# DanieleTeni/Online-Non-Linear-Centroidal-MPC-with-stability-Guarantees-for-Robust-Locomotion-of-Legged-Robots-

Hardware: AMD Instinct MI355X
Metric: centroidal-MPC solves/sec, N=20 horizon (higher is better)
Workload: dtype f64

## Files before the change

build.py:

```python
import os
import subprocess
import sys

ROOT = os.path.dirname(os.path.abspath(__file__))
PKG = os.path.join(ROOT, "online-non-linear-centroidal-mpc-with-stability-guarantees-for-robust-locomotion-of-legged-robots-_amd")


def _newer(target, sources):
    if not os.path.exists(target):
        return True
    t = os.path.getmtime(target)
    return any(os.path.getmtime(s) > t for s in sources)


CSRC = os.path.join(PKG, "csrc")
KERNEL_DEPS = [os.path.join(CSRC, "cmpc_kernel.hpp"), os.path.join(CSRC, "cmpc_lds_asm.hpp"), os.path.join(CSRC, "cmpc_wave.hpp"),
               os.path.join(ROOT, "include", "cmpc.h")]
RBD_DEPS = [os.path.join(CSRC, "rbd_kernel.hpp"), os.path.join(ROOT, "include", "cmpc_rbd.h")]
DEVICE_UNITS = [os.path.join(CSRC, "cmpc_hip.hip"), os.path.join(CSRC, "wbc_qp.hip"), os.path.join(CSRC, "rbd.hip")]
DEVICE_DEPS = DEVICE_UNITS + KERNEL_DEPS + RBD_DEPS + [
    os.path.join(CSRC, "cmpc_order_fit.h"), os.path.join(ROOT, "include", "cmpc_wbc.h")]
EMU_DIR = os.path.join(ROOT, "tests", "emu")


def _hipcc_lib(out, defines=(), force=False, verbose=False):
    if force or _newer(out, DEVICE_DEPS):
        subprocess.check_call(["hipcc"] + (["-Rpass-analysis=kernel-resource-usage"] if verbose else [])
                              + ["--offload-arch=gfx950", "-O3", "-std=c++17", "-fPIC", "-shared"]
                              + ["-D" + d for d in defines] + ["-o", out] + DEVICE_UNITS)
    return out


def _emu_lib(src, out, defines=(), force=False):
    src, out = os.path.join(EMU_DIR, src), os.path.join(EMU_DIR, out)
    if force or _newer(out, [src, os.path.join(EMU_DIR, "cmpc_emu.cpp")] + KERNEL_DEPS):
        subprocess.check_call(["g++", "-O2", "-std=c++17", "-mfma", "-ffp-contract=off", "-fPIC", "-shared", "-pthread"]
                              + ["-D" + d for d in defines] + ["-o", out, src])
    return out


def build_hip(force=False, verbose=False):
    return _hipcc_lib(os.path.join(PKG, "libcmpc_amd.so"), force=force, verbose=verbose)


def build_hip_profile(force=False):
    return _hipcc_lib(os.path.join(ROOT, "tools", "libcmpc_amd_prof.so"), ["CMPC_PROFILE"], force)


def build_hip_dev(force=False):
    return _hipcc_lib(os.path.join(ROOT, "tools", "libcmpc_amd_dev.so"), ["CMPC_DEV_KNOBS"], force)


def build_hip_no_reuse(force=False, profile=False):
    return _hipcc_lib(os.path.join(ROOT, "tools", "libcmpc_amd_noreuse_prof.so" if profile else "libcmpc_amd_noreuse.so"),
                      ["CMPC_NO_EVAL_REUSE", "CMPC_SEPARATE_STEP"] + (["CMPC_PROFILE"] if profile else []), force)


def build_hip_separate_step(force=False, profile=False):
    return _hipcc_lib(os.path.join(ROOT, "tools", "libcmpc_amd_sepstep_prof.so" if profile else "libcmpc_amd_sepstep.so"),
                      ["CMPC_SEPARATE_STEP"] + (["CMPC_PROFILE"] if profile else []), force)


def build_oracle(force=False):
    out = os.path.join(ROOT, "oracle", "libcmpc_oracle.so")
    deps = [os.path.join(ROOT, "oracle", "cmpc_oracle.c"), os.path.join(ROOT, "include", "cmpc.h")]
    if force or _newer(out, deps):
        subprocess.check_call(["make", "-C", os.path.join(ROOT, "oracle"), "-B", "libcmpc_oracle.so"],
                              stdout=subprocess.DEVNULL)
    return out


def build_emu(force=False):
    return _emu_lib("cmpc_emu.cpp", "libcmpc_emu.so", force=force)


def build_emu_gain(force=False):
    return _emu_lib("cmpc_emu_gain.cpp", "libcmpc_emu_gain.so", force=force)


def build_emu_consts(force=False):
    return _emu_lib("cmpc_emu_consts.cpp", "libcmpc_emu_consts.so", force=force)


def build_emu_gain_consts(force=False):
    return _emu_lib("cmpc_emu_gain_consts.cpp", "libcmpc_emu_gain_consts.so", force=force)


def build_emu_reuse(force=False, reuse=True):
    return _emu_lib("cmpc_emu_reuse.cpp", "libcmpc_emu_reuse.so" if reuse else "libcmpc_emu_noreuse.so",
                    [] if reuse else ["CMPC_NO_EVAL_REUSE"], force)


def build_emu_step(force=False, fused=True):
    return _emu_lib("cmpc_emu_step.cpp", "libcmpc_emu_step.so" if fused else "libcmpc_emu_sepstep.so",
                    [] if fused else ["CMPC_SEPARATE_STEP"], force)


def build_emu_rbd(force=False):
    src, out = os.path.join(EMU_DIR, "rbd_emu.cpp"), os.path.join(EMU_DIR, "librbd_emu.so")
    if force or _newer(out, [src] + RBD_DEPS):
        subprocess.check_call(["g++", "-O2", "-std=c++17", "-mfma", "-ffp-contract=off", "-fPIC", "-shared", "-pthread",
                               "-o", out, src])
    return out


def build_device_unit(force=False):
    src = os.path.join(ROOT, "tests", "gpu_unit", "cmpc_device_unit.hip")
    out = os.path.join(ROOT, "tests", "gpu_unit", "libcmpc_device_unit.so")
    if force or _newer(out, [src] + KERNEL_DEPS):
        subprocess.check_call(["hipcc", "--offload-arch=gfx950", "-O3", "-std=c++17", "-fPIC", "-shared", "-o", out, src])
    return out


def build_tools(force=False):
    outs = []
    for name in ("hbm_calib", "lds_b128_repro"):
        src = os.path.join(ROOT, "tools", "ubench", name + ".hip")
        out = os.path.join(ROOT, "tools", "ubench", name)
        if force or _newer(out, [src]):
            r = subprocess.run(["hipcc", "--offload-arch=gfx950", "-O3", "-o", out, src], capture_output=True, text=True)
            if r.returncode != 0:
                print(f"build_tools: {name} failed to compile (profiling scripts that need it will not run)\n{r.stderr}",
                      file=sys.stderr)
                continue
        outs.append(out)
    return outs


if __name__ == "__main__":
    force = "--force" in sys.argv
    print(build_hip(force, verbose="-v" in sys.argv))
    print(build_oracle(force))
    print(build_emu(force))
    print(build_emu_gain(force))
    print(build_emu_consts(force))
    print(build_emu_gain_consts(force))
    print(build_emu_reuse(force))
    print(build_emu_reuse(force, reuse=False))
    print(build_emu_step(force))
    print(build_emu_step(force, fused=False))
    print(build_emu_rbd(force))
    print(build_device_unit(force))
    print(build_tools(force))
```

online-non-linear-centroidal-mpc-with-stability-guarantees-for-robust-locomotion-of-legged-robots-_amd/csrc/cmpc_kernel.hpp:

```cpp
#pragma once
#include "../../include/cmpc.h"
#include <math.h>
#include <utility>
#ifdef CMPC_HOST_EMU
#include <cstdio>
#include <cstdlib>
#endif

#ifndef CMPC_HOST_EMU
#include <hip/hip_runtime.h>
#define CMPC_DEV __device__ __forceinline__
#define CMPC_LANE ((int)threadIdx.x)
#define CMPC_SYNC() asm volatile("s_waitcnt lgkmcnt(0)" ::: "memory")
#define CMPC_SYNC_GLOBAL() __syncthreads()
#define CMPC_SYNC_WG() asm volatile("s_waitcnt lgkmcnt(0)\n\ts_barrier" ::: "memory")
#define CMPC_WAVE_ID() ((int)__builtin_amdgcn_readfirstlane((int)threadIdx.x >> 6))
static __device__ __forceinline__ double cmpc_bcast(double v, int src) {
  union { double d; int i[2]; } u; u.d = v;
  u.i[0] = __builtin_amdgcn_readlane(u.i[0], src);
  u.i[1] = __builtin_amdgcn_readlane(u.i[1], src);
  return u.d;
}
#define CMPC_BCAST(v, src) cmpc_bcast((v), (src))
typedef double cmpc_v4d __attribute__((ext_vector_type(4)));
#define CMPC_MFMA_F64(a, b, c) __builtin_amdgcn_mfma_f64_16x16x4f64((a), (b), (c), 0, 0, 0)
#include "cmpc_wave.hpp"
#define CMPC_PAIR_OF(M, v, a, b) cmpc_pair_of<M>((v), (a), (b))
#define CMPC_OPAQUE(x) asm volatile("" : "+v"(x))
#define CMPC_OPAQUE_D(x) asm volatile("" : "+v"(x))
#define CMPC_OPAQUE_S(x) asm volatile("" : "+s"(x))
#define CMPC_UNIFORM_INT(x) __builtin_amdgcn_readfirstlane(x)
static __device__ __forceinline__ double cmpc_fresh(double a) { asm volatile("" : "+s"(a)); return a; }
#define CMPC_FRESH_D(x) cmpc_fresh(x)
#ifdef CMPC_FRESH_SPEC
#define SPD(field) cmpc_fresh(CMPC_SPEC_OR_ROW(field))
#else
#define SPD(field) (EVAL_REUSE ? cmpc_fresh(CMPC_SPEC_OR_ROW(field)) : CMPC_SPEC_OR_ROW(field))
#endif
typedef const double __attribute__((address_space(4))) *cmpc_crow_t;
#define CMPC_CROW(p) ((cmpc_crow_t)(p))
static __device__ __forceinline__ cmpc_crow_t cmpc_fresh_row(cmpc_crow_t r) { asm volatile("" : "+s"(r)); return r; }
#define CMPC_ROW_AT(r, i) (cmpc_fresh_row(r)[i])
static __device__ __forceinline__ double cmpc_uniform_d(double v) {
  union { double d; int i[2]; } u; u.d = v;
  int lo, hi;
  asm("s_nop 0\n\tv_readfirstlane_b32 %0, %2\n\tv_readfirstlane_b32 %1, %3\n\ts_nop 1" : "=s"(lo), "=s"(hi) : "v"(u.i[0]), "v"(u.i[1]));
  u.i[0] = lo; u.i[1] = hi;
  return u.d;
}
#ifdef CMPC_NO_UNIFORM_D
#define CMPC_UNIFORM_D(x) (x)
#else
#define CMPC_UNIFORM_D(x) cmpc_uniform_d(x)
#endif
#define CMPC_SCHED_FENCE() __builtin_amdgcn_sched_barrier(0)
#define CMPC_RELANE(x) do { (x) = (int)__builtin_amdgcn_mbcnt_hi(~0u, __builtin_amdgcn_mbcnt_lo(~0u, 0u)) + lane_base; } while (0)
#define CMPC_SYNC_WAVE(w) CMPC_SYNC()
#define CMPC_FENCE_WAVE(w) asm volatile("s_waitcnt vmcnt(0) lgkmcnt(0)" ::: "memory")
#define CMPC_VM_LANDED() __builtin_amdgcn_s_waitcnt(0x0F70)
#define CMPC_ASM_NOTE(text) asm volatile("; " text)
#endif
#ifdef CMPC_HOST_EMU
#define CMPC_SYNC_WAVE(w) emu_barrier_wait(&emu_wave_barrier[(w)])
#define CMPC_FENCE_WAVE(w) emu_barrier_wait(&emu_wave_barrier[(w)])
#define CMPC_SYNC_WG() emu_barrier_wait(&emu_barrier)
#define CMPC_VM_LANDED() do { } while (0)
#define CMPC_ASM_NOTE(text) do { } while (0)
#endif
#ifndef CMPC_RELANE
#define CMPC_RELANE(x) do { } while (0)
#define SPD(field) CMPC_SPEC_OR_ROW(field)
typedef const double *cmpc_crow_t;
#define CMPC_CROW(p) ((cmpc_crow_t)(p))
#define CMPC_ROW_AT(r, i) ((r)[i])
#define CMPC_FRESH_D(x) (x)
#define CMPC_UNIFORM_D(x) (x)
#endif
#define CMPC_CIDX(field) ((int)((__builtin_offsetof(cmpc_spec, field) - __builtin_offsetof(cmpc_spec, delta)) / sizeof(double)))
#define CMPC_SPEC_OR_ROW(field) (CONSTS ? CMPC_ROW_AT(crow, CMPC_CIDX(field)) : sp.field)
static_assert(CMPC_CIDX(relax) == CMPC_NCONST - 1 && CMPC_CIDX(box[2]) == 13 && __builtin_offsetof(cmpc_spec, tol) == __builtin_offsetof(cmpc_spec, relax) + sizeof(double),
              "the row of per-instance constants is the block of cmpc_spec from delta to relax");
#define CMPC_FMA(x, y, z) __builtin_fma((x), (y), (z))
#ifdef CMPC_HOST_EMU
#define CMPC_STEP_MAD(t, b, a) ((a) + (t) * (b))
#else
#define CMPC_STEP_MAD(t, b, a) __builtin_fma((t), (b), (a))
#endif
#ifndef CMPC_OPAQUE_D
#define CMPC_OPAQUE_D(x) do { } while (0)
#endif
#ifndef CMPC_UNIFORM_INT
#define CMPC_UNIFORM_INT(x) (x)
#endif
#ifndef CMPC_OPAQUE_S
#define CMPC_OPAQUE_S(x) do { } while (0)
#endif

#if defined(CMPC_PROFILE) && !defined(CMPC_HOST_EMU)
static __device__ __forceinline__ constexpr int cmpc_retry_class(int slot) {
  return (slot == 11 || slot == 12 || slot == 26 || slot == 0) ? 31
       : (slot == 24 || slot == 25) ? 32
       : (slot == 27) ? 34
       : 33;
}
#define CMPC_TICK(slot) do { long long now_ = clock64(); tprof[slot] += now_ - tlast; \
    if (prof_retry) tprof[cmpc_retry_class(slot)] += now_ - tlast; \
    tlast = now_; } while (0)
#define CMPC_TICK_RESET() do { tlast = clock64(); } while (0)
#define CMPC_RETRY_STAT(slot, n) do { tprof[slot] += (n); } while (0)
#define CMPC_RETRY_MARK(on) do { prof_retry = (on); } while (0)
#define CMPC_RETRY_TRACK 1
#else
#define CMPC_TICK(slot) do { } while (0)
#define CMPC_TICK_RESET() do { } while (0)
#define CMPC_RETRY_MARK(on) do { } while (0)
#define CMPC_RETRY_TRACK 0
#endif
#ifndef CMPC_RETRY_STAT
#define CMPC_RETRY_STAT(slot, n) do { } while (0)
#endif
#ifndef CMPC_STEP_STAT
#define CMPC_STEP_STAT(slot, n) do { } while (0)
#endif
#define CMPC_NPROF 36

namespace cmpc {

struct KArgs {
  cmpc_spec sp;
  int B;
  const double *recs;
  const double *warm;
  const double *state_in;
  double *state_out;
  double *out;
  int32_t *status;
  int32_t *iters;
  double *kkt;
  double *scratch;
  size_t scratch_stride;
  long long *prof;
  double tol_acc, tol_tenth;
};

enum { R_LYAP = 0, R_CZ = 1, R_HWC = 2, R_BOX = 3, R_FRIC = 15 };

constexpr double ACC_FACTOR = 100.0;
constexpr int ACC_ITERS = 8;
inline void fill_levels(KArgs &ka) { ka.tol_acc = ACC_FACTOR * ka.sp.tol; ka.tol_tenth = ka.sp.tol / 10; }
constexpr double STALL_STEP = 1e-7;
constexpr int STALL_ITERS = 6;
constexpr int NOPROG_ITERS = 12;
constexpr double PIV_MIN = 1e-8;
constexpr double PIV_FRAC = 0.1;
constexpr int POLISH_ITERS = 1;
constexpr double MU_INIT = 100.0;
constexpr double MU_FACTOR = 0.1;
constexpr double MU_WARM = 1e-7;
constexpr bool COLD_ROLLOUT = true;
constexpr int RESUME_RECENTRE_ITERS = 20;
constexpr int WAVES_NV8 = 2;
constexpr double GAIN_SIG_CAP = 1e12;
constexpr double GAIN_SIG_CAP_BOX = 2e10;

#ifndef CMPC_NO_DEVICE_CODE
#include "cmpc_lds_asm.hpp"
#endif

#ifndef CMPC_NO_DEVICE_CODE
template <int CNT> CMPC_DEV void lds_read_row(double (&v)[CNT], const double *p) {
  static_assert(CNT == 28 || CNT == 32 || CNT == 36 || CNT == 56, "supported row lengths");
  if constexpr (CNT == 28) lds_read_strided28<1>(v, p);
  else if constexpr (CNT == 32) {
    double a[16], b[16];
    lds_read_strided16<1>(a, p); lds_read_strided16<1>(b, p + 16);
#pragma unroll
    for (int i = 0; i < 16; ++i) { v[i] = a[i]; v[16 + i] = b[i]; }
  } else if constexpr (CNT == 36) {
    double a[18], b[18];
    lds_read_strided18<1>(a, p); lds_read_strided18<1>(b, p + 18);
#pragma unroll
    for (int i = 0; i < 18; ++i) { v[i] = a[i]; v[18 + i] = b[i]; }
  } else {
    double a[28], b[28];
    lds_read_strided28<1>(a, p); lds_read_strided28<1>(b, p + 28);
#pragma unroll
    for (int i = 0; i < 28; ++i) { v[i] = a[i]; v[28 + i] = b[i]; }
  }
}
#endif

template <int NV, int NW> struct Sizes {
  static_assert(NW == 1 || NW == 2, "one or two waves per instance");
  static constexpr int WS = 64 * NW;
  static constexpr int NF = 2 * NV;
  static constexpr int NU = 6 * NV + 8;
  static constexpr int NXA = CMPC_NX + 2 * NV;
  static constexpr int NZ = NU + NXA;
  static constexpr int NI = 15 + 10 * NV;
  static constexpr int NTRI = NZ * (NZ + 1) / 2;
  static constexpr int NH = (NZ + WS - 1) / WS;
  static constexpr int PS = NXA + 1;
  static constexpr int LS = NU + 1;
  static constexpr int NPT = NXA * (NXA + 1) / 2;
};

template <int NV, int NW, bool PIPE> struct LdsMap : Sizes<NV, NW> {
// ... 114 lines not shown
  static constexpr int gG = gL + NU;
  static constexpr int gL1 = gG + NI;
  static constexpr int gPV1 = gL1 + NU;
  static constexpr int STAGE = ((gPV1 + NXA + 7) / 8) * 8;
  static constexpr int rH0 = 0, rH1 = rH0 + NZ, rW0 = rH1 + NZ, rVDV = rW0 + NI, rQ = rVDV + 3 * NF, rPI = rQ + 2;
  static constexpr int RE_STAGE = COMPACT ? ((rPI + 3 + 7) / 8) * 8 : 0;
  static constexpr int state_lam(int N) { return CMPC_NSOL(N, NV); }
  static constexpr int state_s(int N) { return state_lam(N) + (N + 1) * NXA; }
  static constexpr int state_z(int N) { return state_s(N) + (N + 1) * NI; }
  static constexpr int state_mu(int N) { return state_z(N) + (N + 1) * NI; }
  static constexpr int state_fl(int N) { return state_mu(N) + 8; }
  static_assert(state_fl(20) + 2 * 21 == CMPC_NSTATE(20, NV), "layout of include/cmpc.h");
  static size_t scratch_doubles(int N) {
    size_t n = (size_t)(N + 1) * STAGE;
    n += (size_t)(N + 1) * NXA * 4;
    n += (size_t)(N + 1) * NU * 3;
    n += (size_t)(N + 1) * NI * 4;
    n += (size_t)(N + 1) * RE_STAGE;
    return (n + 7) / 8 * 8;
  }
};

#ifndef CMPC_NO_DEVICE_CODE

CMPC_DEV int tri(int i) { return i * (i + 1) / 2; }

typedef double cmpc_v2d __attribute__((vector_size(16)));
struct GArr {
  double *p;
  CMPC_DEV double &operator[](unsigned i) const { return *(double *)((char *)p + (size_t)(i * 8u)); }
  CMPC_DEV cmpc_v2d &pair(unsigned i) const { return *(cmpc_v2d *)((char *)p + (size_t)(i * 16u)); }
};

CMPC_DEV bool consts_row_ok(cmpc_crow_t row) {
  bool ok = true;
  for (int i = 0; i < CMPC_NCONST; ++i) {
    const double v = row[i];
    const bool positive = i == CMPC_CIDX(delta) || i == CMPC_CIDX(g) || (i >= CMPC_CIDX(cz_max) && i <= CMPC_CIDX(foot_width));
    const bool gain = i == CMPC_CIDX(k1) || i == CMPC_CIDX(k2);
    ok = ok && v < INFINITY && v > -INFINITY && (positive ? v > 0.0 : (gain || v >= 0.0));
  }
  return ok;
}

template <int NV, int NW = 1, bool PIPE = false, bool GAIN = false, bool CONSTS = false> struct Solver {
  using D = Dims<NV, NW, PIPE>;
  static constexpr int XCH_DU = 16, XCH_DOUBLES = XCH_DU + 2 * D::NU;
  static_assert(!PIPE || XCH_DOUBLES <= D::P_DOUBLES, "the exchange words fit in the unused P region of the second image");
  static constexpr int XCH_AT = D::LDS_DOUBLES + D::oP;
  static_assert(!PIPE || NW == 1, "the pipelined pair runs the one-wave solver");
  static_assert(!PIPE || (D::oUB + 64 <= D::oBV && D::oUB >= D::oXN1 + D::NXA && !D::GT_FIRST),
                "pair_vectors reads BV / writes XN1 of the image the Riccati wave is working in");
  static constexpr int NF = D::NF, NU = D::NU, NXA = D::NXA, NZ = D::NZ, NI = D::NI, NH = D::NH, WS = D::WS;
  static_assert(NW == 1 || NU <= 64, "the input rows (pivot chains, substitutions) live in the first wave");
#ifdef CMPC_NO_EVAL_REUSE
  static constexpr bool EVAL_REUSE = false;
#else
  static constexpr bool EVAL_REUSE = NV == 4 && NW == 1 && !PIPE && !GAIN && D::GT_FIRST;
#endif
  static constexpr bool RETRY_TRACK_POSSIBLE = NV == 4 && NW == 1 && !PIPE && !GAIN;
  static constexpr int ER_AT = 256;
  static_assert(!RETRY_TRACK_POSSIBLE || (ER_AT >= 3 * NZ + NXA + 3 * NF && ER_AT + 6 * WS <= D::NTRI), "the parked error measures fit the M region");
#ifdef CMPC_SEPARATE_STEP
  static constexpr bool STEP_FUSED = false;
#else
  static constexpr bool STEP_FUSED = RETRY_TRACK_POSSIBLE;
#endif
  static constexpr bool RETRY_TRACK = EVAL_REUSE || STEP_FUSED || (CMPC_RETRY_TRACK && NV == 4 && NW == 1 && !PIPE && !GAIN);

  const KArgs &ka;
  const cmpc_spec &sp;
  double *lds;
  double *ldsR;
  int lane_base = 0;
  GArr gs;
  GArr rec;
  int N, lane;
  int wv = 0;
  GArr gx, glam, gdx, glamn, gu, gdu, gupx, gsl, gz, gds, gdz;
  int lr[NH][6];
  double lg[NH][6];
  double piv_min = PIV_MIN;
  GArr st_in{nullptr};
  long long tprof[CMPC_NPROF] = {0, 0, 0, 0, 0, 0, 0, 0, 0, 0, 0, 0, 0, 0, 0, 0, 0, 0, 0, 0, 0, 0, 0, 0, 0, 0, 0, 0, 0, 0, 0, 0, 0, 0, 0, 0}, tlast = 0;
  bool prof_retry = false;
  double *gain_out = nullptr;
  GArr gbuf{nullptr};
  bool gain_sweep = false;
  cmpc_crow_t crow = nullptr;

  CMPC_DEV Solver(const KArgs &a, double *l, double *g, const double *r)
      : ka(a), sp(a.sp), lds(l), ldsR(l), gs{g}, rec{const_cast<double *>(r)}, N(a.sp.N), lane(CMPC_LANE) {
    if constexpr (NW > 1 || PIPE) wv = CMPC_WAVE_ID();
    if constexpr (NW > 1) lane_base = 64 * wv;
    if constexpr (PIPE) lane &= 63;
    if constexpr (NW == 1 && !PIPE) CMPC_RELANE(lane);
    double *p = g + (size_t)(N + 1) * D::STAGE;
    gx = GArr{p}; p += (size_t)(N + 1) * NXA;
    glam = GArr{p}; p += (size_t)(N + 1) * NXA;
    gdx = GArr{p}; p += (size_t)(N + 1) * NXA;
    glamn = GArr{p}; p += (size_t)(N + 1) * NXA;
    gu = GArr{p}; p += (size_t)(N + 1) * NU;
    gdu = GArr{p}; p += (size_t)(N + 1) * NU;
    gupx = GArr{p}; p += (size_t)(N + 1) * NU;
    gsl = GArr{p}; p += (size_t)(N + 1) * NI;
    gz = GArr{p}; p += (size_t)(N + 1) * NI;
    gds = GArr{p}; p += (size_t)(N + 1) * NI;
    gdz = GArr{p};
  }
  CMPC_DEV GArr stage(int k) const { return GArr{gs.p + (size_t)k * D::STAGE}; }
  CMPC_DEV unsigned restage(int k) const {
    CMPC_OPAQUE_S(k);
    return (unsigned)((N + 1 - k) * D::STAGE + (N + 1) * (4 * NXA + 3 * NU + 4 * NI) + k * D::RE_STAGE);
  }
  CMPC_DEV double &L(int o) const { return lds[o]; }
  CMPC_DEV double &R(int o) const { return ldsR[o]; }
  CMPC_DEV void image(int k) { if constexpr (PIPE) lds = ldsR + (k & 1) * D::LDS_DOUBLES; }
  CMPC_DEV void sync() const {
    if constexpr (PIPE) { CMPC_SYNC_WAVE(wv); }
    else {
#ifdef CMPC_HOST_EMU
      CMPC_SYNC();
#else
      if constexpr (NW == 1) CMPC_SYNC(); else CMPC_SYNC_WG();
#endif
    }
  }
  CMPC_DEV void gsync() const {
    if constexpr (PIPE) { CMPC_FENCE_WAVE(wv); } else { CMPC_SYNC_GLOBAL(); }
  }
  CMPC_DEV void pair_sync() const { if constexpr (PIPE) { CMPC_SYNC_GLOBAL(); } }
  CMPC_DEV bool first_wave() const { return NW == 1 || wv == 0; }

  CMPC_DEV double gam_k(int k, int f) const { return (k == N) ? L(D::oHDR + 22 + f) : L(D::oSR + 17 + f); }
  CMPC_DEV double gam_km1(int f) const { return L(D::oSRP + 17 + f); }
  CMPC_DEV void vert_local(int j, double &vx, double &vy) const {
    const double Lh = SPD(foot_length) * 0.5, Wh = SPD(foot_width) * 0.5;
    const double cx[8] = {Lh, Lh, -Lh, -Lh, Lh, 0.0, -Lh, 0.0};
    const double cy[8] = {Wh, -Wh, -Wh, Wh, 0.0, -Wh, 0.0, Wh};
    vx = cx[j]; vy = cy[j];
  }

  CMPC_DEV static double step_axpy(double a, double t, double b) { return CMPC_STEP_MAD(t, b, a); }
  CMPC_DEV static double step_toward(double c, double t, double d) { return CMPC_STEP_MAD(t, d - c, c); }
  CMPC_DEV static void step_slack(double &s, double &z, double ds, double dz, double ap, double ad, double mu) {
    s = CMPC_STEP_MAD(ap, ds, s);
    const double zn = CMPC_STEP_MAD(ad, dz, z);
    const double lo = mu / s / 1e10, hi = mu / s * 1e10;
    z = fmin(fmax(zn, lo), hi);
  }

  CMPC_DEV void load_stage(int k, bool first = false, double mu = 0.0) {
    static_assert(NXA <= 64 && NU <= 64, "one lane per state / input component");
    constexpr int NIH = (NI + WS - 1) / WS;
    const bool in = k < N;
    const int kn = in ? k + 1 : k, ku = in ? k : N - 1, kp = (k >= 1) ? k - 1 : 0;
    const int ix = (lane < NXA) ? lane : 0, iu = (lane < NU) ? lane : 0, ir = (lane < 19) ? lane : 0;
    bool step = false;
    if constexpr (STEP_FUSED) { if (first) step = CMPC_UNIFORM_INT((int)(L(D::oSTEP_ON) != 0.0)) != 0; }
    double dxv = 0.0, lnv = 0.0, duv = 0.0, dsv[NIH], dzv[NIH];
#pragma unroll
    for (int h = 0; h < NIH; ++h) { dsv[h] = 0.0; dzv[h] = 0.0; }
    if constexpr (STEP_FUSED) {
      if (step) {
        dxv = gdx[k * NXA + ix]; lnv = glamn[k * NXA + ix]; duv = gdu[ku * NU + iu];
#pragma unroll
        for (int h = 0; h < NIH; ++h) {
// ... 1293 lines not shown
          if (!riccati_stage(k) && lane == 0) xch[8 + (j & 1)] = 1.0;
        }
        CMPC_SYNC_WG();
        const bool failed = xch[8 + (j & 1)] != 0.0;
        if (failed) { image(0); CMPC_SYNC_WG(); return false; }
      }
      image(0);
      pair_sync();
      return true;
    }
  }

  enum { OP_MAX = 0, OP_MIN = 1, OP_SUM = 2 };
  CMPC_DEV double across_waves(double v, int op) {
    if constexpr (NW == 1) return v;
    if ((lane & 63) == 0) R(D::oCOLD + 4 + wv) = v;
    sync();
    const double a = R(D::oCOLD + 4), b = R(D::oCOLD + 5);
    sync();
    return (op == OP_MAX) ? fmax(a, b) : (op == OP_MIN) ? fmin(a, b) : a + b;
  }
  template <int M> CMPC_DEV static double bfly_sum(double v) { double a, b; CMPC_PAIR_OF(M, v, a, b); return a + b; }
  template <int M> CMPC_DEV static double bfly_max(double v) { double a, b; CMPC_PAIR_OF(M, v, a, b); return fmax(a, b); }
  template <int M> CMPC_DEV static double bfly_min(double v) { double a, b; CMPC_PAIR_OF(M, v, a, b); return fmin(a, b); }
  CMPC_DEV static double wave_sum(double v) {
    v = bfly_sum<32>(v); v = bfly_sum<16>(v); v = bfly_sum<8>(v); v = bfly_sum<4>(v); v = bfly_sum<2>(v); return bfly_sum<1>(v);
  }
  CMPC_DEV double red_max(double v) {
    v = bfly_max<32>(v); v = bfly_max<16>(v); v = bfly_max<8>(v); v = bfly_max<4>(v); v = bfly_max<2>(v); v = bfly_max<1>(v);
    return across_waves(v, OP_MAX);
  }
  CMPC_DEV double red_min(double v) {
    v = bfly_min<32>(v); v = bfly_min<16>(v); v = bfly_min<8>(v); v = bfly_min<4>(v); v = bfly_min<2>(v); v = bfly_min<1>(v);
    return across_waves(v, OP_MIN);
  }
  CMPC_DEV double red_sum(double v) { return across_waves(wave_sum(v), OP_SUM); }

  CMPC_DEV void vector_sweeps(double mu, double dmu, double &ap, double &ad) {
    if constexpr (PIPE) {
      image(0);
      if (wv == 1) { slack_sweep(mu, ap, ad); return; }
    }
    mu = CMPC_UNIFORM_D(mu); dmu = CMPC_UNIFORM_D(dmu);
    const double m = CMPC_UNIFORM_D(rec[20]), muf = CMPC_UNIFORM_D(rec[21]);
    constexpr int NIH = (NI + WS - 1) / WS;
    const double tau = CMPC_UNIFORM_D(fmax(0.99, 1 - mu));
    const double d_m = CMPC_UNIFORM_D(SPD(delta) / m);
    double lap = 1.0, lad = 1.0;
    double *xdu = ldsR + XCH_AT + XCH_DU;
    constexpr bool MERGE = D::W_MERGE;
    const bool isA = lane < NU;
    const int lb = MERGE ? lane - NU : lane;
    const bool isB = lb >= 0 && lb < NXA;
    gsync();
    int cur = D::oXK, nxt = D::oXN1;
    if (lane < NXA) { L(cur + lane) = 0.0; gdx[lane] = 0.0; }
    sync();
    struct Early { double l0v, l1v, dg, pv0, pv1; };
    struct Late { double gh[3][NH], al[NH], sv[NIH], zv[NIH], gv[NIH], hw0, hw1, hw2, bq; };
    double wa[NXA], wb[MERGE ? 1 : NXA], lam[NU];
    auto load_w = [&](int k) {
      const GArr st = stage(k);
      if constexpr (MERGE) {
        const int lc = (lane < NZ) ? lane : 0;
        const int rb = tri(lc) + NU;
#pragma unroll
        for (int c = 0; c < NXA; ++c) wa[c] = st[D::gM + ((lc < NU || NU + c >= lc) ? tri(NU + c) + lc : rb + c)];
        wb[0] = 0.0;
      } else {
        const int la = (lane < NU) ? lane : 0;
        const int lbc = (lane < NXA) ? lane : 0, rb = tri(NU + lbc) + NU;
#pragma unroll
        for (int c = 0; c < NXA; ++c) wa[c] = st[D::gM + tri(NU + c) + la];
#pragma unroll
        for (int c = 0; c < NXA; ++c) wb[c] = st[D::gM + ((c >= lbc) ? tri(NU + c) + NU + lbc : rb + c)];
      }
    };
    auto load_lam = [&](int k) {
      const GArr st = stage(k);
      const int la = (lane < NU) ? lane : 0;
#pragma unroll
      for (int j = 0; j < NU; ++j) lam[j] = st[D::gM + tri(j) + la];
    };
    auto load_early = [&](int k, Early &w) {
      const GArr st = stage(k);
      const int lb_ = MERGE ? lane - NU : lane;
      const int la = (lane < NU) ? lane : 0, lbc = (lb_ >= 0 && lb_ < NXA) ? lb_ : 0;
      w.l0v = st[D::gL + la]; w.l1v = st[D::gL1 + la]; w.dg = st[D::gM + tri(la) + la];
      w.pv0 = st[D::gPV + lbc]; w.pv1 = st[D::gPV1 + lbc];
    };
    auto load_late = [&](int k, Late &w) {
      const GArr st = stage(k);
#pragma unroll
      for (int r = 0; r < 3; ++r)
#pragma unroll
        for (int h = 0; h < NH; ++h) w.gh[r][h] = st[D::gGH + r * D::GHS + lane + WS * h];
      if constexpr (!PIPE) {
#pragma unroll
        for (int h = 0; h < NH; ++h) { const int c = lane + WS * h; w.al[h] = st[D::gAL + ((c < NZ) ? c : 0)]; }
#pragma unroll
        for (int h = 0; h < NIH; ++h) {
          const int r = lane + WS * h, rc = (r < NI) ? r : 0;
          w.sv[h] = gsl[k * NI + rc]; w.zv[h] = gz[k * NI + rc]; w.gv[h] = st[D::gG + rc];
        }
        w.hw0 = gx[k * NXA + 6]; w.hw1 = gx[k * NXA + 7]; w.hw2 = gx[k * NXA + 8];
      } else {
#pragma unroll
        for (int h = 0; h < NH; ++h) w.al[h] = 0.0;
#pragma unroll
        for (int h = 0; h < NIH; ++h) { w.sv[h] = 0.0; w.zv[h] = 0.0; w.gv[h] = 0.0; }
        w.hw0 = 0.0; w.hw1 = 0.0; w.hw2 = 0.0;
      }
      w.bq = st[D::gB + ((lane < NXA) ? lane : 0)];
    };
#ifndef CMPC_FWD_AHEAD_MASK
#define CMPC_FWD_AHEAD_MASK 7
#endif
    constexpr bool AHEAD = ((CMPC_FWD_AHEAD_MASK) >> (PIPE ? 1 : (NW == 1 ? 0 : 2))) & 1;
    Early sm;
    if constexpr (AHEAD) { load_w(0); CMPC_SCHED_FENCE(); load_early(0, sm); CMPC_SCHED_FENCE(); load_lam(0); CMPC_SCHED_FENCE(); }
    else { sm.l0v = 0.0; sm.l1v = 0.0; sm.dg = 0.0; sm.pv0 = 0.0; sm.pv1 = 0.0; }
    for (int k = 0; k <= N; ++k) {
      CMPC_RELANE(lane); CMPC_OPAQUE(lane);
      const bool hasA = k < N, hasB = k >= 1;
      const int kn = hasA ? k + 1 : k;
      const double gl = rec[(k < N) ? 24 + 19 * k + 17 : 22], gr = rec[(k < N) ? 24 + 19 * k + 18 : 23];
      Late lt;
      load_late(k, lt);
      if constexpr (!AHEAD) { load_w(k); load_early(k, sm); load_lam(k); }
      const double (&gh)[3][NH] = lt.gh;
      const double (&al)[NH] = lt.al, (&sv)[NIH] = lt.sv, (&zv)[NIH] = lt.zv, (&gv)[NIH] = lt.gv;
      const double hw0 = lt.hw0, hw1 = lt.hw1, hw2 = lt.hw2, bq = lt.bq;
      const double l0v = sm.l0v, l1v = sm.l1v, dg = sm.dg, pv0 = sm.pv0, pv1 = sm.pv1;
      CMPC_TICK(16);
      double accA, accB;
      {
        const double *dxv = &L(cur);
        double a0 = 0.0, a1 = 0.0, a2 = 0.0, a3 = 0.0;
        static_assert(NXA % 4 == 0, "unroll by 4");
#pragma unroll
        for (int c = 0; c < NXA; c += 4) {
          a0 += wa[c] * dxv[c]; a1 += wa[c + 1] * dxv[c + 1]; a2 += wa[c + 2] * dxv[c + 2]; a3 += wa[c + 3] * dxv[c + 3];
          if (c % 8 == 4) CMPC_SCHED_FENCE();
        }
        accA = (a0 + a1) + (a2 + a3);
        if constexpr (!MERGE) {
          double b0 = 0.0, b1 = 0.0, b2 = 0.0, b3 = 0.0;
#pragma unroll
          for (int c = 0; c < NXA; c += 4) {
            b0 += wb[c] * dxv[c]; b1 += wb[c + 1] * dxv[c + 1]; b2 += wb[c + 2] * dxv[c + 2]; b3 += wb[c + 3] * dxv[c + 3];
          }
          accB = (b0 + b1) + (b2 + b3);
        } else accB = accA;
      }
      CMPC_OPAQUE_D(accA); CMPC_OPAQUE_D(accB);
      if constexpr (AHEAD) load_w(kn);
      if (hasB && isB) glamn[k * NXA + lb] = pv0 + dmu * pv1 + accB;
      auto slack_dirs = [&](double ldot) {
#pragma unroll
        for (int h = 0; h < NIH; ++h) {
          const int r = lane + WS * h;
          if (r < NI) {
            const double sr_ = sv[h], zr = zv[h], gr_ = gv[h];
            double ds = 0.0, dz = 0.0;
            if (zr != 0.0) {
              ds = -(gr_ + sr_) - jg_dot(r, ldot, &L(cur), &L(D::oUK), hw0, hw1, hw2, gl, gr, muf);
              dz = (mu - sr_ * zr - zr * ds) / sr_;
              if (ds < 0) lap = fmin(lap, -tau * sr_ / ds);
              if (dz < 0) lad = fmin(lad, -tau * zr / dz);
            }
            gds[k * NI + r] = ds; gdz[k * NI + r] = dz;
          }
        }
      };
      double duv = 0.0;
      if (hasA && first_wave()) {
        double treg = isA ? -(l0v + dmu * l1v + accA) : 0.0;
        const double dinv = 1.0 / dg;
#pragma unroll
        for (int j = NU - 1; j >= 0; --j) {
          const double dj = CMPC_BCAST(treg * dinv, j);
          if (lane < j) treg -= lam[j] * dj;
        }
        duv = treg * dinv;
        if (isA) { gdu[k * NU + lane] = duv; L(D::oUK + lane) = duv; }
        if constexpr (PIPE) { if (isA) xdu[(k & 1) * NU + lane] = duv; }
      }
      if constexpr (AHEAD) { load_early(kn, sm); load_lam(kn); }
      if (!hasA) {
        if constexpr (PIPE) { CMPC_SYNC_WG(); break; }
        double part = 0.0;
#pragma unroll
        for (int h = 0; h < NH; ++h) {
          const int c = lane + WS * h;
          if (c >= NU && c < NZ) part += al[h] * L(cur + c - NU);
        }
        slack_dirs(red_sum(part));
        sync();
        break;
      }
      if constexpr (PIPE) CMPC_SYNC_WG();
      double s0 = 0.0, s1 = 0.0, s2 = 0.0, s3 = 0.0;
#pragma unroll
      for (int h = 0; h < NH; ++h) {
        const int c = lane + WS * h;
        const bool in = c < NZ;
        const double z = (c < NU) ? duv : (in ? L(cur + c - NU) : 0.0);
        s0 += in ? gh[0][h] * z : 0.0; s1 += in ? gh[1][h] * z : 0.0; s2 += in ? gh[2][h] * z : 0.0;
        if constexpr (!PIPE) s3 += in ? al[h] * z : 0.0;
      }
#define CMPC_STEP4(M) do { s0 = bfly_sum<M>(s0); s1 = bfly_sum<M>(s1); s2 = bfly_sum<M>(s2); if constexpr (!PIPE) s3 = bfly_sum<M>(s3); } while (0)
      CMPC_STEP4(32); CMPC_STEP4(16); CMPC_STEP4(8); CMPC_STEP4(4); CMPC_STEP4(2); CMPC_STEP4(1);
#undef CMPC_STEP4
      if constexpr (NW != 1) {
        if ((lane & 63) == 0) {
          double *w = (wv == 0) ? &L(D::oRED) : &R(D::oCOLD + 4);
          w[0] = s0; w[1] = s1; w[2] = s2; w[3] = s3;
        }
        sync();
        s0 = L(D::oRED) + R(D::oCOLD + 4); s1 = L(D::oRED + 1) + R(D::oCOLD + 5);
        s2 = L(D::oRED + 2) + R(D::oCOLD + 6); s3 = L(D::oRED + 3) + R(D::oCOLD + 7);
      }
      sync();
      if constexpr (!PIPE) slack_dirs(s3);
      CMPC_TICK(17);
      {
        const int q = (lane < NXA) ? lane : 0;
        const double d = SPD(delta);
        const double *dx = &L(cur), *du = &L(D::oUK);
        const int ia = (q < 3) ? 3 + q : ((q >= 9 && q < 12) ? q - 9 : 0), ib = (q >= 9 && q < 12) ? q - 6 : 0;
        const int ja = (q >= CMPC_NX) ? 3 * (q - CMPC_NX) + 2 : (q == 12) ? 6 * NV + 6 : (q >= 13 && q < 16) ? 6 * NV + q - 13
                     : (q == 16) ? 6 * NV + 7 : (q >= 17 && q < 20) ? 6 * NV + 3 + q - 17 : 0;
        const int ax = (q >= 3 && q < 6) ? q - 3 : 0;
        const double own = dx[(q < CMPC_NX) ? q : 0], xa = dx[ia], xb = dx[ib], ua = du[ja];
        double fs = 0.0;
#pragma unroll
        for (int v = 0; v < NF; ++v) fs += ((v < NV) ? gl : gr) * du[3 * v + ax];
        const double gsel = (q >= 16) ? gr : gl;
        const double ssel = (q == 6) ? s0 : (q == 7) ? s1 : s2;
        const double inc = (q < 3) ? own + d * xa : (q < 6) ? own + d_m * fs : (q < 9) ? own + ssel
                         : (q < 12) ? own + d_m * (SPD(k1) * xa + xb) : (q < CMPC_NX) ? own + d * (1 - gsel) * ua : ua;
        const double a = bq + inc;
        if (lane < NXA) {
          gdx[(k + 1) * NXA + q] = a;
          L(nxt + q) = a;
        }
      }
      sync();
      { const int t = cur; cur = nxt; nxt = t; }
      CMPC_TICK(18);
    }
    if constexpr (PIPE) {
      CMPC_SYNC_WG();
      const double *xch = ldsR + XCH_AT;
      ap = xch[6]; ad = xch[7];
    } else {
      ap = red_min(lap); ad = red_min(lad);
    }
  }

  CMPC_DEV void slack_sweep(double mu, double &ap, double &ad) {
    mu = CMPC_UNIFORM_D(mu);
    const double muf = CMPC_UNIFORM_D(rec[21]);
    constexpr int NIH = (NI + WS - 1) / WS;
    const double tau = CMPC_UNIFORM_D(fmax(0.99, 1 - mu));
    double lap = 1.0, lad = 1.0;
    double *xch = ldsR + XCH_AT;
    gsync();
    int cur = D::oXK, nxt = D::oXN1;
    for (int k = 0; k <= N; ++k) {
      const GArr st = stage(k);
      const bool hasA = k < N;
      const double gl = rec[(k < N) ? 24 + 19 * k + 17 : 22], gr = rec[(k < N) ? 24 + 19 * k + 18 : 23];
      double al[NH], sv[NIH], zv[NIH], gv[NIH];
#pragma unroll
      for (int h = 0; h < NH; ++h) { const int c = lane + WS * h; al[h] = st[D::gAL + ((c < NZ) ? c : 0)]; }
#pragma unroll
      for (int h = 0; h < NIH; ++h) {
        const int r = lane + WS * h, rc = (r < NI) ? r : 0;
        sv[h] = gsl[k * NI + rc]; zv[h] = gz[k * NI + rc]; gv[h] = st[D::gG + rc];
      }
      const double hw0 = gx[k * NXA + 6], hw1 = gx[k * NXA + 7], hw2 = gx[k * NXA + 8];
      CMPC_SYNC_WG();
      const double *du = xch + XCH_DU + (k & 1) * NU;
      double ldot = 0.0;
#pragma unroll
      for (int h = 0; h < NH; ++h) {
        const int c = lane + WS * h;
        const bool in = c < NZ;
        if (hasA) {
          const double z = (c < NU) ? du[(c < NU) ? c : 0] : (in ? L(cur + c - NU) : 0.0);
          ldot += in ? al[h] * z : 0.0;
        } else if (c >= NU && c < NZ) ldot += al[h] * L(cur + c - NU);
      }
      ldot = wave_sum(ldot);
#pragma unroll
      for (int h = 0; h < NIH; ++h) {
        const int r = lane + WS * h;
        if (r < NI) {
          const double sr_ = sv[h], zr = zv[h], gr_ = gv[h];
          double ds = 0.0, dz = 0.0;
          if (zr != 0.0) {
            ds = -(gr_ + sr_) - jg_dot(r, ldot, &L(cur), du, hw0, hw1, hw2, gl, gr, muf);
            dz = (mu - sr_ * zr - zr * ds) / sr_;
            if (ds < 0) lap = fmin(lap, -tau * sr_ / ds);
            if (dz < 0) lad = fmin(lad, -tau * zr / dz);
          }
          gds[k * NI + r] = ds; gdz[k * NI + r] = dz;
        }
      }
      { const int t = cur; cur = nxt; nxt = t; }
    }
    ap = red_min(lap); ad = red_min(lad);
    if (lane == 0) { xch[6] = ap; xch[7] = ad; }
    CMPC_SYNC_WG();
  }

  CMPC_DEV double jg_dot(int r, double lyap_dot, const double *dx, const double *du, double hw0, double hw1, double hw2,
                         double g0, double g1, double muf) const {
    const bool is_box = r >= R_BOX && r < R_FRIC, is_fr = r >= R_FRIC;
    const int qb = is_box ? r - R_BOX : 0, fb = qb / 6, ab = (qb % 6) / 2;
    const int qf = is_fr ? r - R_FRIC : 0, v = qf / 5, t = qf % 5;
    const double d2 = dx[2], d6 = dx[6], d7 = dx[7], d8 = dx[8], dbx = dx[13 + 4 * fb + ab];
    const double fx = du[3 * v], fy = du[3 * v + 1], fz = du[3 * v + 2];
    const int sgn = (qb & 1) ? -1 : 1;
    const double v_box = sgn * (fb ? g1 : g0) * dbx;
    const double gg = (v / NV) ? g1 : g0;
    const double v_fr = (t == 0) ? gg * (fx - muf * fz) : (t == 1) ? gg * (-fx - muf * fz) : (t == 2) ? gg * (fy - muf * fz)
                      : (t == 3) ? gg * (-fy - muf * fz) : -gg * fz;
    const double v_hw = 2.0 * (hw0 * d6 + hw1 * d7 + hw2 * d8);
    return (r == R_LYAP) ? lyap_dot : (r == R_CZ) ? d2 : (r == R_HWC) ? v_hw : (is_box ? v_box : v_fr);
// ... 498 lines not shown
```

Baseline: 92330.

## Prefetch next node's late words and split Lambda loads in forward sweep

In the single-wave, non-pipelined forward sweep, the late-stage words (gh, al, slack vectors, bq) for the next node are now loaded during the current iteration, and the Lambda column load is split into two halves issued at different points. This hides global-load latency behind the current node's state update. The glamn and gdu stores are moved so they do not wait on the new loads, and the last iteration is restructured to break after the sync. It also adds forward-only profiling slots and build variants that keep the old late-at-top schedule. In exchange it uses more live registers for the prefetched Late struct and makes the loop control more complex.

```diff
diff --git a/build.py b/build.py
--- a/build.py
+++ b/build.py
@@ -43,8 +43,9 @@
     return _hipcc_lib(os.path.join(PKG, "libcmpc_amd.so"), force=force, verbose=verbose)
 
 
-def build_hip_profile(force=False):
-    return _hipcc_lib(os.path.join(ROOT, "tools", "libcmpc_amd_prof.so"), ["CMPC_PROFILE"], force)
+def build_hip_profile(force=False, forward_only=False):
+    return _hipcc_lib(os.path.join(ROOT, "tools", "libcmpc_amd_prof_fwd.so" if forward_only else "libcmpc_amd_prof.so"),
+                      ["CMPC_PROFILE"] + (["CMPC_PROFILE_FWD"] if forward_only else []), force)
 
 
 def build_hip_dev(force=False):
@@ -59,6 +60,12 @@
 def build_hip_separate_step(force=False, profile=False):
     return _hipcc_lib(os.path.join(ROOT, "tools", "libcmpc_amd_sepstep_prof.so" if profile else "libcmpc_amd_sepstep.so"),
                       ["CMPC_SEPARATE_STEP"] + (["CMPC_PROFILE"] if profile else []), force)
+
+
+def build_hip_late_at_top(force=False, profile=False, forward_only=False):
+    name = "libcmpc_amd_latetop" + ("_prof_fwd" if profile and forward_only else "_prof" if profile else "") + ".so"
+    return _hipcc_lib(os.path.join(ROOT, "tools", name), ["CMPC_FWD_LATE_AT_TOP"] + (["CMPC_PROFILE"] if profile else [])
+                      + (["CMPC_PROFILE_FWD"] if profile and forward_only else []), force)
 
 
 def build_oracle(force=False):
@@ -94,6 +101,10 @@
 def build_emu_step(force=False, fused=True):
     return _emu_lib("cmpc_emu_step.cpp", "libcmpc_emu_step.so" if fused else "libcmpc_emu_sepstep.so",
                     [] if fused else ["CMPC_SEPARATE_STEP"], force)
+
+
+def build_emu_late_at_top(force=False):
+    return _emu_lib("cmpc_emu.cpp", "libcmpc_emu_latetop.so", ["CMPC_FWD_LATE_AT_TOP"], force)
 
 
 def build_emu_rbd(force=False):
@@ -139,6 +150,7 @@
     print(build_emu_reuse(force, reuse=False))
     print(build_emu_step(force))
     print(build_emu_step(force, fused=False))
+    print(build_emu_late_at_top(force))
     print(build_emu_rbd(force))
     print(build_device_unit(force))
     print(build_tools(force))
diff --git a/online-non-linear-centroidal-mpc-with-stability-guarantees-for-robust-locomotion-of-legged-robots-_amd/csrc/cmpc_kernel.hpp b/online-non-linear-centroidal-mpc-with-stability-guarantees-for-robust-locomotion-of-legged-robots-_amd/csrc/cmpc_kernel.hpp
--- a/online-non-linear-centroidal-mpc-with-stability-guarantees-for-robust-locomotion-of-legged-robots-_amd/csrc/cmpc_kernel.hpp
+++ b/online-non-linear-centroidal-mpc-with-stability-guarantees-for-robust-locomotion-of-legged-robots-_amd/csrc/cmpc_kernel.hpp
@@ -103,18 +103,26 @@
        : (slot == 27) ? 34
        : 33;
 }
+#ifdef CMPC_PROFILE_FWD
+#define CMPC_TICK_SLOT(slot) (((slot) == 16 || (slot) == 17 || (slot) == 18 || (slot) == 36) ? (slot) : 37)
+#define CMPC_TICK(slot) do { long long now_ = clock64(); tprof[CMPC_TICK_SLOT(slot)] += now_ - tlast; tlast = now_; } while (0)
+#define CMPC_RETRY_STAT(slot, n) do { } while (0)
+#else
 #define CMPC_TICK(slot) do { long long now_ = clock64(); tprof[slot] += now_ - tlast; \
     if (prof_retry) tprof[cmpc_retry_class(slot)] += now_ - tlast; \
     tlast = now_; } while (0)
+#define CMPC_RETRY_STAT(slot, n) do { tprof[slot] += (n); } while (0)
+#endif
 #define CMPC_TICK_RESET() do { tlast = clock64(); } while (0)
-#define CMPC_RETRY_STAT(slot, n) do { tprof[slot] += (n); } while (0)
 #define CMPC_RETRY_MARK(on) do { prof_retry = (on); } while (0)
 #define CMPC_RETRY_TRACK 1
+#define CMPC_PROFILED 1
 #else
 #define CMPC_TICK(slot) do { } while (0)
 #define CMPC_TICK_RESET() do { } while (0)
 #define CMPC_RETRY_MARK(on) do { } while (0)
 #define CMPC_RETRY_TRACK 0
+#define CMPC_PROFILED 0
 #endif
 #ifndef CMPC_RETRY_STAT
 #define CMPC_RETRY_STAT(slot, n) do { } while (0)
@@ -122,7 +130,7 @@
 #ifndef CMPC_STEP_STAT
 #define CMPC_STEP_STAT(slot, n) do { } while (0)
 #endif
-#define CMPC_NPROF 36
+#define CMPC_NPROF 38
 
 namespace cmpc {
 
@@ -403,7 +411,7 @@
   double lg[NH][6];
   double piv_min = PIV_MIN;
   GArr st_in{nullptr};
-  long long tprof[CMPC_NPROF] = {0, 0, 0, 0, 0, 0, 0, 0, 0, 0, 0, 0, 0, 0, 0, 0, 0, 0, 0, 0, 0, 0, 0, 0, 0, 0, 0, 0, 0, 0, 0, 0, 0, 0, 0, 0}, tlast = 0;
+  long long tprof[CMPC_NPROF] = {}, tlast = 0;
   bool prof_retry = false;
   double *gain_out = nullptr;
   GArr gbuf{nullptr};
@@ -1863,6 +1871,12 @@
 #pragma unroll
       for (int j = 0; j < NU; ++j) lam[j] = st[D::gM + tri(j) + la];
     };
+    auto load_lam_half = [&](int k, const int j0) {
+      const GArr st = stage(k);
+      const int la = (lane < NU) ? lane : 0;
+#pragma unroll
+      for (int i = NU / 2 - 1; i >= 0; --i) lam[j0 + i] = st[D::gM + tri(j0 + i) + la];
+    };
     auto load_early = [&](int k, Early &w) {
       const GArr st = stage(k);
       const int lb_ = MERGE ? lane - NU : lane;
@@ -1870,7 +1884,7 @@
       w.l0v = st[D::gL + la]; w.l1v = st[D::gL1 + la]; w.dg = st[D::gM + tri(la) + la];
       w.pv0 = st[D::gPV + lbc]; w.pv1 = st[D::gPV1 + lbc];
     };
-    auto load_late = [&](int k, Late &w) {
+    auto load_late_main = [&](int k, Late &w) {
       const GArr st = stage(k);
 #pragma unroll
       for (int r = 0; r < 3; ++r)
@@ -1892,26 +1906,43 @@
         for (int h = 0; h < NIH; ++h) { w.sv[h] = 0.0; w.zv[h] = 0.0; w.gv[h] = 0.0; }
         w.hw0 = 0.0; w.hw1 = 0.0; w.hw2 = 0.0;
       }
-      w.bq = st[D::gB + ((lane < NXA) ? lane : 0)];
     };
+    auto load_bq = [&](int k, Late &w) { w.bq = stage(k)[D::gB + ((lane < NXA) ? lane : 0)]; };
+    auto load_late = [&](int k, Late &w) { load_late_main(k, w); load_bq(k, w); };
 #ifndef CMPC_FWD_AHEAD_MASK
 #define CMPC_FWD_AHEAD_MASK 7
 #endif
     constexpr bool AHEAD = ((CMPC_FWD_AHEAD_MASK) >> (PIPE ? 1 : (NW == 1 ? 0 : 2))) & 1;
+#ifndef CMPC_FWD_LATE_MASK
+#ifdef CMPC_FWD_LATE_AT_TOP
+#define CMPC_FWD_LATE_MASK 0
+#else
+#define CMPC_FWD_LATE_MASK 3
+#endif
+#endif
+    constexpr bool LATE_WORDS = AHEAD && NW == 1 && !PIPE && !GAIN && ((CMPC_FWD_LATE_MASK) & 1);
+    constexpr bool LAM_HALVES = AHEAD && NW == 1 && !PIPE && !GAIN && ((CMPC_FWD_LATE_MASK) & 2);
+    constexpr bool LATE_AHEAD = LATE_WORDS || LAM_HALVES;
+    static_assert(!LATE_AHEAD || NU % 2 == 0, "Lambda's column in two halves");
     Early sm;
-    if constexpr (AHEAD) { load_w(0); CMPC_SCHED_FENCE(); load_early(0, sm); CMPC_SCHED_FENCE(); load_lam(0); CMPC_SCHED_FENCE(); }
+    Late lt;
+    if constexpr (LATE_AHEAD) {
+      load_w(0); CMPC_SCHED_FENCE(); load_early(0, sm); CMPC_SCHED_FENCE();
+      if constexpr (LAM_HALVES) { load_lam_half(0, NU / 2); CMPC_SCHED_FENCE(); load_lam_half(0, 0); CMPC_SCHED_FENCE(); }
+      else { load_lam(0); CMPC_SCHED_FENCE(); }
+      if constexpr (LATE_WORDS) { load_late_main(0, lt); CMPC_SCHED_FENCE(); load_bq(0, lt); CMPC_SCHED_FENCE(); }
+    } else if constexpr (AHEAD) { load_w(0); CMPC_SCHED_FENCE(); load_early(0, sm); CMPC_SCHED_FENCE(); load_lam(0); CMPC_SCHED_FENCE(); }
     else { sm.l0v = 0.0; sm.l1v = 0.0; sm.dg = 0.0; sm.pv0 = 0.0; sm.pv1 = 0.0; }
     for (int k = 0; k <= N; ++k) {
       CMPC_RELANE(lane); CMPC_OPAQUE(lane);
       const bool hasA = k < N, hasB = k >= 1;
       const int kn = hasA ? k + 1 : k;
-      const double gl = rec[(k < N) ? 24 + 19 * k + 17 : 22], gr = rec[(k < N) ? 24 + 19 * k + 18 : 23];
-      Late lt;
-      load_late(k, lt);
+      double gl = rec[(k < N) ? 24 + 19 * k + 17 : 22], gr = rec[(k < N) ? 24 + 19 * k + 18 : 23];
+      if constexpr (!LATE_WORDS) load_late(k, lt);
       if constexpr (!AHEAD) { load_w(k); load_early(k, sm); load_lam(k); }
       const double (&gh)[3][NH] = lt.gh;
       const double (&al)[NH] = lt.al, (&sv)[NIH] = lt.sv, (&zv)[NIH] = lt.zv, (&gv)[NIH] = lt.gv;
-      const double hw0 = lt.hw0, hw1 = lt.hw1, hw2 = lt.hw2, bq = lt.bq;
+      const double &hw0 = lt.hw0, &hw1 = lt.hw1, &hw2 = lt.hw2, &bq = lt.bq;
       const double l0v = sm.l0v, l1v = sm.l1v, dg = sm.dg, pv0 = sm.pv0, pv1 = sm.pv1;
       CMPC_TICK(16);
       double accA, accB;
@@ -1935,8 +1966,10 @@
         } else accB = accA;
       }
       CMPC_OPAQUE_D(accA); CMPC_OPAQUE_D(accB);
+      if constexpr (LATE_AHEAD) { if (hasB && isB) glamn[k * NXA + lb] = pv0 + dmu * pv1 + accB; }
+      if constexpr (NW == 1 && !PIPE && !GAIN) CMPC_ASM_NOTE("cmpc: forward sweep, Ls | P of the next node");
       if constexpr (AHEAD) load_w(kn);
-      if (hasB && isB) glamn[k * NXA + lb] = pv0 + dmu * pv1 + accB;
+      if constexpr (!LATE_AHEAD) { if (hasB && isB) glamn[k * NXA + lb] = pv0 + dmu * pv1 + accB; }
       auto slack_dirs = [&](double ldot) {
 #pragma unroll
         for (int h = 0; h < NIH; ++h) {
@@ -1964,10 +1997,25 @@
           if (lane < j) treg -= lam[j] * dj;
         }
         duv = treg * dinv;
-        if (isA) { gdu[k * NU + lane] = duv; L(D::oUK + lane) = duv; }
+        if (isA) { if constexpr (!LATE_AHEAD) gdu[k * NU + lane] = duv; L(D::oUK + lane) = duv; }
         if constexpr (PIPE) { if (isA) xdu[(k & 1) * NU + lane] = duv; }
       }
-      if constexpr (AHEAD) { load_early(kn, sm); load_lam(kn); }
+      if constexpr (LAM_HALVES) { load_early(kn, sm); load_lam_half(kn, NU / 2); }
+      else if constexpr (AHEAD) { load_early(kn, sm); load_lam(kn); }
+      if constexpr (NW == 1 && !PIPE && !GAIN) {
+        CMPC_TICK(17);
+        CMPC_ASM_NOTE("cmpc: forward sweep, the wait for the late words");
+        if constexpr (LATE_AHEAD) { CMPC_OPAQUE_D(gr); CMPC_OPAQUE_D(gl); CMPC_OPAQUE_D(lt.bq); }
+        if constexpr (CMPC_PROFILED) {
+#pragma unroll
+          for (int h = 0; h < NH; ++h) { CMPC_OPAQUE_D(lt.gh[0][h]); CMPC_OPAQUE_D(lt.gh[1][h]); CMPC_OPAQUE_D(lt.gh[2][h]); CMPC_OPAQUE_D(lt.al[h]); }
+#pragma unroll
+          for (int h = 0; h < NIH; ++h) { CMPC_OPAQUE_D(lt.sv[h]); CMPC_OPAQUE_D(lt.zv[h]); CMPC_OPAQUE_D(lt.gv[h]); }
+          CMPC_OPAQUE_D(lt.hw0); CMPC_OPAQUE_D(lt.hw1); CMPC_OPAQUE_D(lt.hw2);
+        }
+        CMPC_TICK(36);
+        if constexpr (LATE_AHEAD) { if (hasA && first_wave() && isA) gdu[k * NU + lane] = duv; }
+      }
       if (!hasA) {
         if constexpr (PIPE) { CMPC_SYNC_WG(); break; }
         double part = 0.0;
@@ -1977,35 +2025,42 @@
           if (c >= NU && c < NZ) part += al[h] * L(cur + c - NU);
         }
         slack_dirs(red_sum(part));
+        if constexpr (!LATE_AHEAD) {
+          sync();
+          break;
+        }
+      }
+      if constexpr (PIPE) CMPC_SYNC_WG();
+      double s0 = 0.0, s1 = 0.0, s2 = 0.0;
+      if (!LATE_AHEAD || hasA) {
+        double s3 = 0.0;
+#pragma unroll
+        for (int h = 0; h < NH; ++h) {
+          const int c = lane + WS * h;
+          const bool in = c < NZ;
+          const double z = (c < NU) ? duv : (in ? L(cur + c - NU) : 0.0);
+          s0 += in ? gh[0][h] * z : 0.0; s1 += in ? gh[1][h] * z : 0.0; s2 += in ? gh[2][h] * z : 0.0;
+          if constexpr (!PIPE) s3 += in ? al[h] * z : 0.0;
+        }
+#define CMPC_STEP4(M) do { s0 = bfly_sum<M>(s0); s1 = bfly_sum<M>(s1); s2 = bfly_sum<M>(s2); if constexpr (!PIPE) s3 = bfly_sum<M>(s3); } while (0)
+        CMPC_STEP4(32); CMPC_STEP4(16); CMPC_STEP4(8); CMPC_STEP4(4); CMPC_STEP4(2); CMPC_STEP4(1);
+#undef CMPC_STEP4
+        if constexpr (NW != 1) {
+          if ((lane & 63) == 0) {
+            double *w = (wv == 0) ? &L(D::oRED) : &R(D::oCOLD + 4);
+            w[0] = s0; w[1] = s1; w[2] = s2; w[3] = s3;
+          }
+          sync();
+          s0 = L(D::oRED) + R(D::oCOLD + 4); s1 = L(D::oRED + 1) + R(D::oCOLD + 5);
+          s2 = L(D::oRED + 2) + R(D::oCOLD + 6); s3 = L(D::oRED + 3) + R(D::oCOLD + 7);
+        }
         sync();
-        break;
-      }
-      if constexpr (PIPE) CMPC_SYNC_WG();
-      double s0 = 0.0, s1 = 0.0, s2 = 0.0, s3 = 0.0;
-#pragma unroll
-      for (int h = 0; h < NH; ++h) {
-        const int c = lane + WS * h;
-        const bool in = c < NZ;
-        const double z = (c < NU) ? duv : (in ? L(cur + c - NU) : 0.0);
-        s0 += in ? gh[0][h] * z : 0.0; s1 += in ? gh[1][h] * z : 0.0; s2 += in ? gh[2][h] * z : 0.0;
-        if constexpr (!PIPE) s3 += in ? al[h] * z : 0.0;
-      }
-#define CMPC_STEP4(M) do { s0 = bfly_sum<M>(s0); s1 = bfly_sum<M>(s1); s2 = bfly_sum<M>(s2); if constexpr (!PIPE) s3 = bfly_sum<M>(s3); } while (0)
-      CMPC_STEP4(32); CMPC_STEP4(16); CMPC_STEP4(8); CMPC_STEP4(4); CMPC_STEP4(2); CMPC_STEP4(1);
-#undef CMPC_STEP4
-      if constexpr (NW != 1) {
-        if ((lane & 63) == 0) {
-          double *w = (wv == 0) ? &L(D::oRED) : &R(D::oCOLD + 4);
-          w[0] = s0; w[1] = s1; w[2] = s2; w[3] = s3;
-        }
-        sync();
-        s0 = L(D::oRED) + R(D::oCOLD + 4); s1 = L(D::oRED + 1) + R(D::oCOLD + 5);
-        s2 = L(D::oRED + 2) + R(D::oCOLD + 6); s3 = L(D::oRED + 3) + R(D::oCOLD + 7);
-      }
-      sync();
-      if constexpr (!PIPE) slack_dirs(s3);
+        if constexpr (!PIPE) slack_dirs(s3);
+      }
       CMPC_TICK(17);
-      {
+      if constexpr (LAM_HALVES) load_lam_half(kn, 0);
+      if constexpr (LATE_WORDS) load_late_main(kn, lt);
+      if (!LATE_AHEAD || hasA) {
         const int q = (lane < NXA) ? lane : 0;
         const double d = SPD(delta);
         const double *dx = &L(cur), *du = &L(D::oUK);
@@ -2027,7 +2082,9 @@
           L(nxt + q) = a;
         }
       }
+      if constexpr (LATE_WORDS) load_bq(kn, lt);
       sync();
+      if constexpr (LATE_AHEAD) { if (!hasA) break; }
       { const int t = cur; cur = nxt; nxt = t; }
       CMPC_TICK(18);
     }
```

Measured after the change: 92930, median of 6. About the same (+0.6%).
